# Lecanyu/SparsifyPoseGraph

Measured on AMD Instinct MI355X. Metric: nodes_marginalized_per_s, higher is better.
Workload: dtype f64

## Files before the change

sparsifyposegraph_amd/csrc/spg_graph_impl.h:

```cpp
#pragma once
#include <algorithm>
#include <atomic>
#include <chrono>
#include <cmath>
#include <cstdio>
#include <cstdlib>
#include <cstring>
#include <set>
#include <string>
#include <thread>
#if defined(__linux__)
#include <pthread.h>
#include <sched.h>
#endif
#include <unistd.h>
#include <unordered_map>
#include <unordered_set>
#include <vector>
#include "../../include/spg.h"
#include "spg_internal.h"

namespace {
inline int pose_stride(int d) { return d == 3 ? 3 : 7; }
inline int info_len(int d) { return d * (d + 1) / 2; }
// ... 86 lines not shown
    spg_backend be{};
    bool is_hip = false;
    int rank = 0, nranks = 1;
    void *rccl = nullptr;
    int tag_counter = 0;
    int linear_solver = 0;
    double pcg_rel_tol = 0;
    int pcg_max_iter = 0;
    spg_pcg_stats pcg_stats{};
    spg::StreamPort *sim_port = nullptr;
    char err[768] = {0};
};

struct GEdge {
    int64_t off;
    int64_t key;
    int32_t len;
    int32_t vtx[2];
    int16_t nv;
    int8_t kind;
    uint8_t alive;
};

struct RoundBlanket {
    int32_t root;
    int32_t n_remove;
    int32_t vbeg = 0, nv = 0;
    int32_t ebeg = 0, ne = 0;
    int32_t rank = 0;
    int32_t owner = -1;
    spg_blanket_desc desc{};
};

struct BlanketLog { int32_t root_id, round, status, info; double kld, min_gap; };

struct Batch {
    std::vector<RoundBlanket> rb;
    std::vector<int32_t> rb_verts, rb_edges;
    std::vector<spg_blanket_desc> h_blk;
    std::vector<int64_t> h_vpo;
    std::vector<spg_edge_ref> h_er;
    std::vector<int32_t> h_ev;
    std::vector<int64_t> chunk_hdr;
    spg_round_info rinfo{};
    bool round_open = false;
    bool used_mailbox = false;
// ... 22 lines not shown
        if (vdirect_ok) return (id >= 0 && (size_t)id < vdirect.size()) ? vdirect[(size_t)id] : -1;
        auto it = vidx.find(id);
        return it == vidx.end() ? -1 : it->second;
    }
    std::vector<uint8_t> valive;
    std::vector<int64_t> vpose;
    struct AdjEnt { int32_t eid, other; operator int32_t() const { return eid; } };
    struct SVtx {
        int32_t nown;
        int32_t own[4];
        int32_t slot;
    };
    struct alignas(64) VRec {
        InlVec<AdjEnt, 7> adj;
        SVtx s;
        int32_t id, pad_;
        int64_t pose;
        char spare_[24];
        VRec() { s.nown = 0; s.slot = -1; id = 0; pad_ = 0; pose = 0; }
    };
    std::vector<VRec> vr;
    std::vector<InlVec<struct OwnRefT, 3>> vown;
    std::vector<int32_t> cst;
    std::vector<GEdge> edges;
    std::vector<int32_t> everts;
    int n_live_v = 0, n_live_e = 0;
    void *dev = nullptr;
    int64_t cap = 0, used = 0;
    HostMirror host;
    int64_t dev_synced = 0;
    int64_t stale_lo = 0, stale_hi = 0;
    bool active = false;
    spg_options opts{};
    int rank = 0, nranks = 1;
    std::vector<int32_t> pending;
    size_t pend_head = 0;
    std::vector<uint8_t> in_set;
    static constexpr int NB = 8;
    Batch bt[NB];
    Batch *B = &bt[0];
    struct Owner { int32_t batch, off, len; uint32_t gen; };
    using OwnRef = OwnRefT;
    std::vector<Owner> owners;
    std::vector<int32_t> owner_free, transient;
    std::vector<int32_t> Dpool;
    int shard_threshold = -1;
    int round_no = 0, launch_seq = 0;
    bool pipelined = false;
    spg_marg_stats stats{};
    double tr_age = 0, tr_wait = 0, tr_first = 0; long tr_n = 0;
    std::vector<BlanketLog> log;
    std::vector<double> hdr_buf;
    std::thread sub_thread;
    static constexpr uint32_t SUBQ = 8;
    bool sub_active = false;
    struct alignas(64) SubShared {
        alignas(64) std::atomic<uint32_t> tail{0};
        alignas(64) Batch *q[SUBQ] = {nullptr};
        alignas(64) std::atomic<uint32_t> head{0};
        alignas(64) double seconds = 0;
// ... 3 lines not shown
    std::vector<int32_t> live_rank;
    long n_mutations = 0, live_rank_stamp = -1;
    int64_t next_key = 0, key_base = 0;
    static constexpr int64_t kKeyStride = 65536;
    std::vector<int32_t> lpos;
    std::vector<int32_t> vstamp, estamp;
    int32_t stamp = 0;
    std::vector<int32_t> ocnt;
    std::vector<int32_t> lidx;
    std::vector<int32_t> s_newpending, s_B, s_centres, s_Dv, s_tmp, s_work, s_seen, s_hit, s_vix;
    std::vector<double> s_cost;
    std::vector<int> s_first;
    static constexpr int kSOwn = 4, kSMaxV = 16, kSMaxE = 44;
    struct SSlot {
        int32_t pos, root, nv, ne, n_new_max, tag, logi, bell;
        int32_t launched;
        int32_t npend, pend[3];
        int32_t mcell;
        int64_t new_off, out_off;
        int32_t verts[kSMaxV];
        int32_t edges[kSMaxE];
    };
    std::vector<SSlot> sslots;
    std::vector<int32_t> s_free, s_fifo, s_fin, s_woken, s_ready, wl_next, wl_stable, wl_done;
    int64_t unsorted_from = -1;
    bool layout_diverged = false;
    int stream_emulation = -1;
    int stream_disabled = 0;
};

static inline const int32_t *edge_verts(const spg_graph *g, const GEdge &e) {
    return e.nv == 2 ? e.vtx : g->everts.data() + e.vtx[0];
}

inline int set_err(spg_ctx *c, int code, const char *fmt, const char *a = "") {
    if (c) snprintf(c->err, sizeof c->err, fmt, a);
    return code;
}

int sync_host(spg_graph *g);
int sync_device(spg_graph *g);
void canonicalize_edge_order(spg_graph *g);
#pragma GCC visibility push(hidden)
int arena_ensure(spg_graph *g, int64_t need);
int add_edge_idx(spg_graph *g, int kind, int nv, const int32_t *vix, int64_t off, int32_t len, int64_t key = -1);
void quiesce_submission(spg_graph *g);
int stream_marginalize(spg_graph *g, bool *started = nullptr);
#pragma GCC visibility pop

namespace {
inline void next_stamp(spg_graph *g) {
    if (g->vstamp.size() < g->vid.size()) g->vstamp.resize(g->vid.size(), 0);
    if (g->estamp.size() < g->edges.size()) g->estamp.resize(g->edges.size(), 0);
    g->stamp++;
}

inline void mark_stale(spg_graph *g, int64_t lo, int64_t hi) {
    if (g->stale_hi <= g->stale_lo) { g->stale_lo = lo; g->stale_hi = hi; }
    else { g->stale_lo = std::min(g->stale_lo, lo); g->stale_hi = std::max(g->stale_hi, hi); }
}

inline void copy_backend_error(spg_ctx *c) { snprintf(c->err, sizeof c->err, "%s", spg::hip_backend_error(&c->be)); }

enum MailState { MAIL_NOT_YET = 0, MAIL_READY = 1, MAIL_FINAL = 2 };
inline MailState mail_state(double word, double tag) {
    return word == SPG_READY_WORD(tag) ? MAIL_READY : word == SPG_FINAL_WORD(tag) ? MAIL_FINAL : MAIL_NOT_YET;
}

inline bool out_record_well_formed(const double *rec, const spg_blanket_desc &bd, int nv) {
// ... 81 lines not shown
```

sparsifyposegraph_amd/csrc/spg_hip_backend.cpp:

```cpp
#include <hip/hip_runtime.h>
#include <atomic>
#include <chrono>
#include <cstdio>
#include <cstdlib>
#include <cstring>
#include <vector>
#include <algorithm>
#include "../../include/spg.h"
#include "spg_blanket_layout.hpp"
#include "spg_hip_buffers.hpp"
#include "spg_internal.h"
#include "spg_round_plan.hpp"

namespace spg {

#define HIPCHK(x) do { hipError_t e_ = (x); if (e_ != hipSuccess) { snprintf(err, (size_t)512, "%s:%d %s -> %s", __FILE__, __LINE__, #x, hipGetErrorString(e_)); return SPG_EHIP; } } while (0)

namespace {

bool env_is(const char *name, char c) { const char *e = getenv(name); return e && e[0] == c; }

struct HipBackend {
    int device = 0;
    char err[512] = {0};
// ... 5 lines not shown
        PinnedBuf stage;
        bool busy = false;
        RoundPlan plan;
        hipEvent_t done = nullptr, wait_ev = nullptr;
        DevBuf bar;
        std::vector<const volatile double *> finals;
        double final_word = 0;
        DevBuf pkt;
        bool stream_dirty = false;
        std::vector<Timed> pending;
        std::vector<std::pair<hipEvent_t, hipEvent_t>> pool;
        double prof_ms = 0, prof_bytes = 0;
        long long prof_launches = 0, prof_blankets = 0;
    };
    static constexpr int NSLOT = 8;
    Slot slots[NSLOT];
    struct Worker {
        hipStream_t stream = nullptr;
        DevBuf qmem;
        DevBuf ticket;
        WorkQ *q() const { return (WorkQ *)qmem.p; }
        hipEvent_t ev_a = nullptr, ev_b = nullptr;
        bool running = false, disabled = false;
        int D = 0, alg = 0;
        unsigned long long tail = 0;
        double bytes = 0;
        long long blankets = 0;
        int bells = 1, lazy = 0;
        int wgs = 256;
        std::chrono::steady_clock::time_point last_push;
    } worker;
    int batches_in_call = 0;
    DevBuf st_pkt;
    PinnedBuf st_mail;
    int worker_cooldown = 0;
    double prof_big_ms = 0, prof_big_flops = 0;
    long long prof_big_count = 0;
    int prof_big_nmax = 0;
    double prof_worker_ms = 0, prof_worker_bytes = 0;
    long long prof_worker_runs = 0, prof_worker_blankets = 0;
    int lds_limit = 160 * 1024;
    bool large_bar = false;
    std::atomic<int> n_launches{0};
    const bool force_one_wave = env_is("SPG_ONE_WAVE", '1');
    const bool worker_env = !env_is("SPG_WORKER", '0');
    const bool worker_stamp = env_is("SPG_WORKER_STAMP", '1');
// ... 92 lines not shown
        t.bytes = B.bytes; t.blankets = nblocks;
    }
    const hipEvent_t stop = timed ? t.b : S.done;
    if (int rc = hip_blanket_launch(B.variant, S.stream, timed ? t.a : nullptr, stop, ka, nblocks, B.lds, err, sizeof err)) {
        if (timed) S.pool.push_back({t.a, t.b});
        return rc;
    }
    if (timed) S.pending.push_back(t);
    S.wait_ev = stop;
    n_launches++;
    S.stream_dirty = true;
    return 0;
}

inline void bar_fence() {
    std::atomic_thread_fence(std::memory_order_release);
#if defined(__x86_64__)
    __builtin_ia32_sfence();
#endif
}

int HipBackend::worker_start(int D, int alg) {
    Worker &W = worker;
    if (W.running && W.D == D && W.alg == alg) {
        if (std::chrono::duration<double>(std::chrono::steady_clock::now() - W.last_push).count() < 1.0) return 0;
    }
    if (W.running) if (int rc = worker_stop()) return rc;
    if (!W.stream) {
        HIPCHK(hipStreamCreateWithFlags(&W.stream, hipStreamNonBlocking));
        HIPCHK(hipEventCreate(&W.ev_a));
        HIPCHK(hipEventCreate(&W.ev_b));
        if (W.qmem.alloc_fine(sizeof(WorkQ)) != hipSuccess) { (void)hipGetLastError(); W.disabled = true; return 1; }
        HIPCHK(W.ticket.alloc(64));
        const char *e = getenv("SPG_WORKER_WGS");
        if (e && atoi(e) > 0) W.wgs = atoi(e);
        if ((e = getenv("SPG_WORKER_BELLS")) && atoi(e) >= 1 && atoi(e) <= kBells) W.bells = atoi(e);
        if ((e = getenv("SPG_WORKER_LAZY")) && atoi(e) >= 0) W.lazy = atoi(e);
    }
    WorkQ *q = W.q();
    for (int c = 0; c < W.bells; c++) q->tail[c * kBellStride] = 0;
    q->stop = 0;
    bar_fence();
    W.tail = 0; W.bytes = 0; W.blankets = 0;
    HIPCHK(hipMemsetAsync(W.ticket.p, 0, 64, W.stream));
    Layout L = make_layout(D, 128, kWorkerMaxN / D, 1, alg, SPG_TOPO_TREE, 0);
    const size_t lds = (size_t)(L.small_doubles + L.mat_doubles) * 8;
    const long long idle_ticks = 10LL * 100000000LL;
    if (int rc = hip_worker_launch(D, W.wgs, lds, W.stream, W.ev_a, W.ev_b, q, (unsigned long long *)W.ticket.p, idle_ticks, W.bells, W.lazy, err, sizeof err)) return rc;
    W.running = true; W.D = D; W.alg = alg;
    W.last_push = std::chrono::steady_clock::now();
    n_launches++;
    return 0;
}

int HipBackend::worker_stop() {
    Worker &W = worker;
    if (!W.running) return 0;
    W.q()->stop = 1;
    bar_fence();
    HIPCHK(hipStreamSynchronize(W.stream));
    W.running = false;
    if (profiling) {
        float ms = 0;
        if (hipEventElapsedTime(&ms, W.ev_a, W.ev_b) == hipSuccess) {
            prof_worker_ms += ms; prof_worker_bytes += W.bytes; prof_worker_runs++; prof_worker_blankets += W.blankets;
        }
    }
    return 0;
}

int HipBackend::push_to_worker(Slot &S, const spg_round_desc *rd, void *arena) {
    const spg_options &o = *rd->opts;
    const int D = o.pose_dim;
    const size_t n_push = (size_t)rd->count;
    bool fine = true;
    if (int rc = ensure_fine(S.pkt, n_push * (size_t)kPktWords * 8, (size_t)512 * kPktWords * 8, &fine)) return rc;
    if (!fine) worker.disabled = true;
    if (int rc = ensure_pinned(S.mail, (size_t)rd->mail_len * 8, true)) return rc;
    if (worker.disabled) return 1;
    if (int wrc = worker_start(D, SPG_ALG_NFR)) return wrc;
    Worker &W = worker;
    WorkQ *q = W.q();
    unsigned long long *pbase = (unsigned long long *)S.pkt.p;
    const double *hmail = (const double *)S.mail.h;
// ... 200 lines not shown
        double secs = 0, flops = 0;
        const int info_bits = (rd->opts->flags & SPG_FLAG_GLC_KLD) ? SPG_INFO_GLC_KLD_SKIPPED : 0;
        if (int brc = hip_big_glc_dense((void *)S.stream, g.in, m, k, Nm, bd.new_off, orec, bd.n_new_max, rd->tag, info_bits, &secs, &flops, err, sizeof err)) return brc;
        prof_big_ms += 1e3 * secs; prof_big_flops += flops; prof_big_count++;
        prof_big_nmax = std::max(prof_big_nmax, D * (k + m));
        S.wait_ev = nullptr;
        S.stream_dirty = true;
    }
    return 0;
}

int HipBackend::run_round(void *arena, const spg_round_desc *rd) {
    if (rd->count <= 0) return 0;
    Slot &S = slots[rd->slot & (NSLOT - 1)];
    const spg_options &o = *rd->opts;
    if (o.pose_dim != 3 && o.pose_dim != 6) return SPG_EINVAL;
    if (int rc = make_current()) return rc;
    if (S.busy) if (int rc = wait_slot(S)) return rc;
    drain_profile(S);
    S.busy = true;
    PlanConfig cfg;
    cfg.lds_limit = lds_limit; cfg.force_one_wave = force_one_wave; cfg.large_bar = large_bar;
    cfg.worker_enabled = worker_env && !worker.disabled; cfg.force_big = force_big; cfg.profiling = profiling;
    const WorkerState ws{++batches_in_call, worker_cooldown, worker.running};
    plan_worker(rd, cfg, ws, S.plan);
    worker_cooldown = S.plan.cooldown;
    if (S.plan.to_worker) {
        const int rc = push_to_worker(S, rd, arena);
        if (rc <= 0) return rc;
    }
    if (int rc = worker_stop()) return rc;
    if (int rc = plan_launch(rd, cfg, S.plan, err, sizeof err)) return rc;
    Staged sd{};
    if (int rc = stage_descriptors(S, rd, sd)) return rc;
    double *mail_dev = nullptr;
    if (rd->mail_len > 0) {
        if (int rc = ensure_pinned(S.mail, (size_t)rd->mail_len * 8, true)) return rc;
        mail_dev = (double *)S.mail.d;
    }
    KArgs ka;
    ka.arena = (double *)arena;
    ka.blk = (const spg_blanket_desc *)(sd.base + sd.o_blk);
    ka.vpo = (const int64_t *)(sd.base + sd.o_vpo);
    ka.er = (const spg_edge_ref *)(sd.base + sd.o_er);
    ka.ev = (const int32_t *)(sd.base + sd.o_ev);
    ka.list = nullptr;
    ka.mail = mail_dev;
// ... 176 lines not shown
    if (wrc) return wrc;
    if (hb->worker.disabled) return 1;
    hb->batches_in_call += 3;
    out->pkt = (unsigned long long *)hb->st_pkt.p;
    out->q = hb->worker.q();
    out->tail = hb->worker.tail;
    out->bells = hb->worker.bells;
    out->h_mail = (const double *)hb->st_mail.h;
    out->d_mail = (unsigned long long)(uintptr_t)hb->st_mail.d;
    out->mail_stride = mail_stride;
    out->slots = slots;
    return 0;
}

void hip_stream_close(spg_backend *b, const StreamPort *port, double alg_bytes, long long blankets) {
    HipBackend *hb = (HipBackend *)b->user;
    if (!hb || !port) return;
    hb->worker.tail = port->tail;
    hb->worker.bytes += alg_bytes;
    hb->worker.blankets += blankets;
    hb->worker.last_push = std::chrono::steady_clock::now();
}

}
```

sparsifyposegraph_amd/csrc/spg_host_rounds.cpp:

```cpp
#include "spg_graph_impl.h"

static void closed_neighbourhood(spg_graph *g, int32_t v, std::vector<int32_t> &out) {
    next_stamp(g);
    out.clear();
    out.push_back(v);
    g->vstamp[v] = g->stamp;
    for (int32_t eid : g->vr[v].adj) {
        const GEdge &e = g->edges[eid];
        for (int i = 0; i < e.nv; i++) {
            int32_t u = edge_verts(g, e)[i];
            if (g->vstamp[u] != g->stamp) { g->vstamp[u] = g->stamp; out.push_back(u); }
        }
    }
}

static void extended_blanket(spg_graph *g, int32_t root, std::vector<int32_t> &verts, std::vector<int32_t> &picked) {
    auto byid = [g](int32_t a, int32_t b) { return g->vid[a] < g->vid[b]; };
    std::set<int32_t, decltype(byid)> ret(byid), pk(byid);
    std::vector<int32_t> tmp;
    closed_neighbourhood(g, root, tmp);
    ret.insert(tmp.begin(), tmp.end());
    pk.insert(root);
    for (auto it = ret.begin(); it != ret.end(); ++it) {
        int32_t v = *it;
// ... 182 lines not shown
                    }
                }
            }
            if (Dv.size() > DCAP) { stop = true; continue; }
            {
                int32_t off = (int32_t)g->Dpool.size();
                g->Dpool.insert(g->Dpool.end(), Dv.begin(), Dv.end());
                g->transient.push_back(reg(-1, off, (int32_t)Dv.size()));
            }
            static const int pat_inflight = [] { const char *e = getenv("SPG_PATIENCE"); return e ? atoi(e) : 16; }();
            size_t patience = inflight ? pat_inflight + bt.rb.size() / 16 : 48 + bt.rb.size() / 8;
            if (++consec > patience || n_deferred > 256 + 2 * bt.rb.size()) stop = true;
            PT(3);
        }
    }
    {
        size_t nd = newpending.size();
        size_t nh = pos - nd;
        for (size_t i = 0; i < nd; i++) g->pending[nh + i] = newpending[i];
        g->pend_head = nh;
    }
}

extern "C" int spg_graph_marginalize_begin(spg_graph *g, const int32_t *which, int n, const spg_options *opts, int rank, int nranks) {
    if (!g || !opts || (n > 0 && !which) || nranks < 1 || rank < 0 || rank >= nranks) return SPG_EINVAL;
    if (g->active) return set_err(g->ctx, SPG_ESTATE, "marginalize already in progress");
    if (opts->pose_dim != g->d) return set_err(g->ctx, SPG_EINVAL, "pose_dim mismatch");
    g->opts = *opts;
    g->rank = rank; g->nranks = nranks;
    g->pending.clear();
    g->pend_head = 0;
    g->in_set.assign(g->vid.size(), 0);
    g->lpos.assign(g->vid.size(), -1);
    for (int i = 0; i < n; i++) {
        const int32_t vi = g->index_of(which[i]);
        if (vi < 0 || !g->valive[vi])
            return set_err(g->ctx, SPG_EINVAL, "vertex needs to exist in order to be marginalized");
        if (g->in_set[vi]) continue;
        g->in_set[vi] = 1;
        g->lpos[vi] = (int32_t)g->pending.size();
        g->pending.push_back(vi);
    }
    g->key_base = g->next_key;
    g->next_key = g->key_base + ((int64_t)g->pending.size() + 1) * spg_graph::kKeyStride;
    if (g->cap < g->used * 5 / 2 + (1 << 16)) if (int rc = arena_ensure(g, g->used * 3 + (1 << 20))) return rc;
    if (int rc = sync_device(g)) return rc;
    g->active = true;
    for (int i = 0; i < spg_graph::NB; i++) { g->bt[i].round_open = false; g->bt[i].slot = i; }
    g->B = &g->bt[0];
    g->round_no = 0;
    g->launch_seq = 0;
    g->pipelined = false;
    g->stats = spg_marg_stats{};
    g->log.clear();
    return 0;
}

extern "C" int spg_graph_set_shard_threshold(spg_graph *g, int min_blankets) {
    if (!g) return SPG_EINVAL;
    g->shard_threshold = min_blankets < 0 ? -1 : min_blankets;
    return 0;
}

static bool shard_pays(const spg_graph *g, const Batch &bt) {
    const int B = (int)bt.rb.size(), nr = g->nranks;
    if (nr <= 1 || B == 0) return false;
    if (g->shard_threshold >= 0) return B >= g->shard_threshold;
    const int d = g->d;
    double t_sum = 0, t_max = 0, bytes = 0;
    for (const RoundBlanket &r : bt.rb) {
        const double n = (double)d * (r.nv - r.n_remove), nm = (double)d * r.n_remove;
        const double tb = 45e-6 * std::pow(std::max(1.0, n / 24.0), 2.5);
        const double lds = 8.0 * (3 * n * n + nm * nm + nm * n) + 4096.0;
        const double per_cu = lds > 160.0 * 1024 ? 1.0 : std::min(6.0, std::floor(160.0 * 1024 / lds));
        t_sum += tb / (256.0 * per_cu);
        t_max = std::max(t_max, tb);
        int32_t nn, nvv; int64_t nl;
        new_edge_budget(g->opts, d, r.nv - r.n_remove, nn, nvv, nl);
// ... 344 lines not shown
            return set_err(g->ctx, SPG_EHIP, "%s", msg);
        }
        const int64_t key0 = g->key_base + (int64_t)g->lpos[r.root] * spg_graph::kKeyStride;
        for_each_new_edge(rec, n_new, bd.n_new_max, [&](int e, int kind, int64_t rel, int32_t len, int nv, const double *lv) {
            vix.resize(nv);
            for (int i = 0; i < nv; i++) vix[i] = rverts[(int)lv[i]];
            add_edge_idx(g, kind, nv, vix.data(), bd.new_off + rel, len, key0 + e);
            g->stats.n_new_edges++;
        });
        PT(10);
    }
    bt.round_open = false;
    release_batch_owners(g, bt);
    g->stats.n_rounds = g->round_no;
    g->stats.host_seconds += now_s() - t1;
    g->stats.commit_seconds += now_s() - t1;
    return 0;
}

extern "C" int spg_graph_marginalize_end(spg_graph *g, spg_marg_stats *stats) {
    if (!g || !g->active) return SPG_ESTATE;
    submission_stop(g);
    g->active = false;
    for (int i = 0; i < spg_graph::NB; i++) (void)harvest_kld(g, g->bt[i]);
    for (int i = 0; i < spg_graph::NB; i++) { g->bt[i].round_open = false; release_batch_owners(g, g->bt[i]); g->bt[i].rb.clear(); }
    for (int32_t oid : g->transient) owner_release(g, oid);
    g->transient.clear();
    g->B = &g->bt[0];
    if (g->ctx->is_hip) (void)spg::hip_backend_end_of_call(&g->ctx->be);
    if (g->tr_n && getenv("SPG_TRACE"))
        fprintf(stderr, "spg trace: %ld batches; per batch: launch call -> commit start %.1f us, wait for the ready words %.1f us (launch call -> first blanket ready %.1f us)\n",
                g->tr_n, 1e6 * g->tr_age / g->tr_n, 1e6 * g->tr_wait / g->tr_n, 1e6 * g->tr_first / g->tr_n);
    g->tr_n = 0; g->tr_age = g->tr_wait = g->tr_first = 0;
    if (g->ctx->is_hip) g->stats.n_launches = spg::hip_backend_launches(&g->ctx->be);
#ifdef SPG_SCHED_PROF
    if (getenv("SPG_SCHED_PROF")) {
        const char *nm[12] = {"neighbourhood", "owner scan", "select:reg", "defer", "-", "select:sort", "select:edges", "commit:log", "commit:rm edges", "commit:rm verts", "commit:add", "prepare"};
        for (int i = 0; i < 12; i++) { fprintf(stderr, "sched %-14s %10llu calls %8.3f Mcycles\n", nm[i], prof_n[i], prof_t[i] * 1e-6); prof_t[i] = prof_n[i] = 0; }
    }
#endif
    if (stats) *stats = g->stats;
    return g->stats.n_bad_status ? SPG_EBLANKET : 0;
}

static Batch *oldest_open_batch(spg_graph *g) {
    Batch *o = nullptr;
// ... 7 lines not shown
    for (size_t i = from; i < to; i++) {
        RoundBlanket r = a.rb[i];
        int32_t vb = (int32_t)b.rb_verts.size(), eb = (int32_t)b.rb_edges.size();
        b.rb_verts.insert(b.rb_verts.end(), a.rb_verts.begin() + r.vbeg, a.rb_verts.begin() + r.vbeg + r.nv);
        b.rb_edges.insert(b.rb_edges.end(), a.rb_edges.begin() + r.ebeg, a.rb_edges.begin() + r.ebeg + r.ne);
        r.vbeg = vb; r.ebeg = eb;
        if (r.owner >= 0) { g->owners[r.owner].batch = bidx; g->owners[r.owner].off = vb; }
        b.rb.push_back(r);
    }
}

extern "C" int spg_graph_marginalize(spg_graph *g, const int32_t *which, int n, const spg_options *opts, spg_marg_stats *stats) {
    return spg_graph_marginalize_ranks(g, which, n, opts, 0, 1, nullptr, nullptr, stats);
}

extern "C" int spg_graph_marginalize_ranks(spg_graph *g, const int32_t *which, int n, const spg_options *opts, int rank, int nranks,
                                           spg_exchange_fn exchange, void *exchange_user, spg_marg_stats *stats) {
    if (!g) return SPG_EINVAL;
    const bool builtin = nranks > 1 && !exchange;
    if (builtin && (!g->ctx->rccl || g->ctx->nranks != nranks || g->ctx->rank != rank))
        return set_err(g->ctx, SPG_EINVAL, "spg_graph_marginalize_ranks: no exchange callback and the context has no matching RCCL communicator (spg_ctx_create_ranks)");
    int launches0 = (g && g->ctx->is_hip) ? spg::hip_backend_launches(&g->ctx->be) : 0;
    const double t_call = now_s();
    int rc = spg_graph_marginalize_begin(g, which, n, opts, rank, nranks);
    if (rc) return rc;
    const double t_begun = now_s();
    const char *env = getenv("SPG_NO_PIPELINE");
    g->pipelined = g->ctx->be.synchronize_slot && g->ctx->be.mailbox_slot && !(env && env[0] == '1');
    int stream_rc = 1;
    if (nranks == 1 && !exchange) stream_rc = stream_marginalize(g);
    else if (nranks > 1) {
        bool independent = g->layout_diverged;
        if (!independent && g->shard_threshold < 0) {
            const std::vector<int32_t> saved = g->pending;
            g->B = &g->bt[0];
            schedule_round(g);
            independent = !g->bt[0].rb.empty() && !shard_pays(g, g->bt[0]);
            release_batch_owners(g, g->bt[0]);
            g->bt[0].rb.clear(); g->bt[0].rb_verts.clear(); g->bt[0].rb_edges.clear();
            for (int32_t oid : g->transient) owner_release(g, oid);
            g->transient.clear();
            g->pending = saved;
            g->pend_head = 0;
        }
        if (independent) {
            const int rank0 = g->rank, nranks0 = g->nranks;
            g->rank = 0; g->nranks = 1;
            bool started = false;
            stream_rc = stream_marginalize(g, &started);
            if (started || g->layout_diverged) g->layout_diverged = true;
            else { g->rank = rank0; g->nranks = nranks0; }
        }
    }
    if (stream_rc <= 0) {
        const double t_streamed = now_s();
        int rc2 = spg_graph_marginalize_end(g, stats);
        if (getenv("SPG_TRACE")) fprintf(stderr, "spg trace: marginalize: begin %.3f ms, stream %.3f ms, end %.3f ms\n", 1e3 * (t_begun - t_call), 1e3 * (t_streamed - t_begun), 1e3 * (now_s() - t_streamed));
        if (stats && g->ctx->is_hip) stats->n_launches -= launches0;
        return stream_rc < 0 ? stream_rc : rc2;
    }
    auto do_exchange = [&](Batch &b) -> int {
        if (!b.rinfo.exchange) return 0;
        double tx = now_s();
        int erc = g->ctx->be.synchronize(g->ctx->be.user);
        if (erc) return erc;
        erc = builtin ? spg_allgather_region(g->ctx, g->dev, b.rinfo.region_off, b.rinfo.chunk_len)
                      : exchange(exchange_user, g->dev, b.rinfo.region_off, b.rinfo.chunk_len, g->nranks, g->rank);
        g->stats.n_exchanged++;
        g->stats.exchanged_bytes += 8.0 * (double)b.rinfo.chunk_len * g->nranks;
        g->stats.exchange_seconds += now_s() - tx;
        return erc;
    };
    if (!g->pipelined) {
        for (;;) {
            rc = spg_graph_round_prepare(g, nullptr);
            if (rc <= 0) break;
// ... 88 lines not shown
```

sparsifyposegraph_amd/csrc/spg_host_stream.cpp:

```cpp
#include "spg_graph_impl.h"

#if defined(__x86_64__)
#include <x86intrin.h>
static inline uint64_t ticks_now() { return __rdtsc(); }
#else
static inline uint64_t ticks_now() { return (uint64_t)(now_s() * 1e9); }
#endif

namespace {
enum : uint8_t { SV_WAITING = 0, SV_STABLE = 1, SV_INFLIGHT = 2, SV_DONE = 3 };
constexpr int kStreamSlots = 2048;
constexpr int kStreamMailStride = 8;

__attribute__((always_inline)) inline void unregister_blanket(spg_graph *g, const int32_t s) {
    const spg_graph::SSlot &sl = g->sslots[s];
    spg_graph::VRec *const vr = g->vr.data();
    for (int i = 0; i < sl.nv; i++) {
        spg_graph::SVtx &sx = vr[sl.verts[i]].s;
        for (int j = 0; j < sx.nown; j++) if (sx.own[j] == s) { sx.own[j] = sx.own[--sx.nown]; break; }
    }
}

struct Streamer {
    spg_graph *g;
    const bool emulate;
    const int D, ps, rec;
    const int32_t P;
    int32_t cursor = 0;
    int32_t prefetched_to = 0;
    int32_t n_done = 0, n_inflight = 0, pending_bell = 0, bell_no = 0;
    bool fallback = false;
    int32_t cap_wait = -1;
    uint64_t t_idle = 0;

    Streamer(spg_graph *g_, bool emu) : g(g_), emulate(emu), D(g_->d), ps(g_->ps), rec(g_->rec), P((int32_t)g_->pending.size()), arena_dev(g_->dev) {}

    struct SvView { spg_graph::VRec *vr; spg_graph::SVtx &operator[](int32_t i) const { return vr[i].s; } };

    long n_exam = 0, n_park[8] = {0};
    const bool prof = [] { const char *e = getenv("SPG_STREAM_PROF"); return e && e[0] == '1'; }();
    uint64_t pt[8] = {0}, pn[8] = {0}, pt_last = 0;
    inline void P0() { if (prof) pt_last = ticks_now(); }
    inline void P1(int i) { if (prof) { const uint64_t n = ticks_now(); pt[i] += n - pt_last; pn[i]++; pt_last = n; } }
    void park(std::vector<int32_t> &heads, int32_t on, int32_t p) { g->wl_next[p] = heads[on]; heads[on] = p; }
    void wake(std::vector<int32_t> &heads, int32_t on) {
        for (int32_t p = heads[on]; p >= 0;) { const int32_t nx = g->wl_next[p]; g->s_woken.push_back(p); p = nx; }
        heads[on] = -1;
    }

    static inline int find(const int32_t *X, const int nX, const int32_t y) { for (int i = 0; i < nX; i++) if (X[i] == y) return i; return -1; }
    static inline void adj_remove(InlVec<spg_graph::AdjEnt, 7> &av, const int32_t eid) {
        for (size_t j = 0; j < av.size(); j++) if (av[j].eid == eid) { av[j] = av.back(); av.pop_back(); break; }
    }
    inline void set_pend(spg_graph::SSlot &sl, const int32_t *X, const int nX) {
        const int32_t *const cst = g->cst.data();
        sl.npend = 0;
        for (int i = 1; i < nX; i++) if (cst[X[i]] >= 0) { if (sl.npend == 3) { sl.npend = -1; break; } sl.pend[sl.npend++] = X[i]; }
    }
    __attribute__((always_inline)) inline void register_blanket(const int32_t s, const int32_t p, const int32_t *X, const int nX) {
        const SvView sv{g->vr.data()};
        spg_graph::SSlot &sl = g->sslots[s];
        sl.pos = p; sl.root = X[0]; sl.nv = nX;
        memcpy(sl.verts, X, sizeof(int32_t) * (size_t)nX);
        set_pend(sl, X, nX);
        for (int i = 0; i < nX; i++) { spg_graph::SVtx &sx = sv[X[i]]; sx.own[sx.nown++] = s; }
    }

    void reserve(const int32_t p, const int32_t *X, const int nX) {
// ... 324 lines not shown
            uint32_t q = poll_seq;
            for (int n = 0; q != launch_seq && n < 12; q++) {
                if (cell_slot[q & mask] < 0) continue;
                __builtin_prefetch((const void *)(port.h_mail + (size_t)(q & mask) * (size_t)port.mail_stride));
                n++;
            }
        }
    }

    struct Helper {
        static constexpr uint32_t RQ = 4096;
        alignas(64) std::atomic<uint32_t> launches{0};
        alignas(64) std::atomic<uint32_t> r_tail{0};
        alignas(64) std::atomic<int> stop{0};
        alignas(64) uint32_t r_head = 0;
        std::vector<double> rq;
        std::vector<uint32_t> cell_tag;
        char pad_[64];
    } hp;
    bool helper = false;
    std::thread helper_thread;
    std::vector<const double *> ready_rec;

    void helper_main() {
        const uint32_t mask = (uint32_t)(port.slots - 1);
        std::vector<uint8_t> pend((size_t)port.slots, 0);
        uint32_t head = 0, seen = 0, r_tail = 0;
        unsigned n = 0;
        while (!hp.stop.load(std::memory_order_acquire)) {
            const uint32_t lp = hp.launches.load(std::memory_order_acquire);
            while (seen != lp) { pend[seen & mask] = 1; seen++; }
            while (head != seen && !pend[head & mask]) head++;
            const int giveup = (++n & 15) ? 10 : 1 << 20;
            bool got = false;
            scan_mailbox(head, seen, giveup,
                         [&](uint32_t cell, double &tagd) -> int32_t {
                             if (!pend[cell]) return -1;
                             tagd = (double)hp.cell_tag[cell];
                             return (int32_t)cell;
                         },
                         [&](uint32_t q, int32_t cell, bool final) {
                             double *e = hp.rq.data() + (size_t)(r_tail & (Helper::RQ - 1)) * 8;
                             memcpy(e, port.h_mail + (size_t)cell * (size_t)port.mail_stride, 64);
                             e[5] = (double)(2.0 * (double)q + (final ? 1.0 : 0.0));
                             r_tail++;
                             pend[cell] = 0;
                             got = true;
                         });
            if (got) hp.r_tail.store(r_tail, std::memory_order_release);
        }
    }
    void take_helper_results() {
        const uint32_t rt = hp.r_tail.load(std::memory_order_acquire);
        const uint32_t mask = (uint32_t)(port.slots - 1);
        ready_rec.clear();
        while (hp.r_head != rt) {
            const double *e = hp.rq.data() + (size_t)(hp.r_head & (Helper::RQ - 1)) * 8;
            __builtin_prefetch(e + 8); __builtin_prefetch(e + 16);
            const uint32_t q = (uint32_t)((uint64_t)e[5] >> 1);
            const int32_t s = cell_slot[q & mask];
            g->s_ready.push_back(s);
            ready_rec.push_back(e);
            cell_slot[q & mask] = -2;
            __builtin_prefetch(&g->sslots[s]); __builtin_prefetch((const char *)&g->sslots[s] + 64); __builtin_prefetch((const char *)&g->sslots[s] + 128);
            hp.r_head++;
        }
    }
    bool helper_start() {
#if defined(__linux__)
        static const bool pin = [] { const char *e = getenv("SPG_PIN_THREADS"); return !(e && e[0] == '0'); }();
        if (!pin || sched_getaffinity(0, sizeof old_mask, &old_mask) != 0) return false;
        const int cpu = sched_getcpu();
        int cand = -1;
        for (int d = 1; cpu >= 0 && d < 8 && cand < 0; d++) {
            const int c = (cpu & ~7) | ((cpu + d) & 7);
            if (c < CPU_SETSIZE && CPU_ISSET(c, &old_mask)) cand = c;
        }
        if (cand < 0) return false;
        cpu_set_t one; CPU_ZERO(&one); CPU_SET(cpu, &one);
        if (sched_setaffinity(0, sizeof one, &one) != 0) return false;
        repin = true;
        hp.rq.resize((size_t)Helper::RQ * 8);
        hp.cell_tag.assign((size_t)port.slots, 0);
        helper = true;
        helper_thread = std::thread([this] { helper_main(); });
        CPU_ZERO(&one); CPU_SET(cand, &one);
        (void)pthread_setaffinity_np(helper_thread.native_handle(), sizeof one, &one);
        return true;
#else
        return false;
#endif
    }
    void helper_stop() {
        if (!helper) return;
        hp.stop.store(1, std::memory_order_release);
        helper_thread.join();
        helper = false;
#if defined(__linux__)
        if (repin) (void)sched_setaffinity(0, sizeof old_mask, &old_mask);
#endif
    }
#if defined(__linux__)
    cpu_set_t old_mask;
    bool repin = false;
#endif

    size_t fifo_head = 0;
    uint64_t rng;
// ... 152 lines not shown
        const double s_begin = now_s();
        last_progress = t_begin;
        for (;;) {
            if (int r = take_results()) return r;
            const bool got = !ready.empty();
            if (got && idle_since) { t_idle += ticks_now() - idle_since; idle_since = 0; }
            commit_ready();
            examine_woken();
            late_results();
            advance_cursor(got);
            ring();
            if (n_done == P) break;
            if (fallback && n_inflight == 0) break;
            if (got || cursor < P) { last_progress = ticks_now(); continue; }
            if (int r = idle_check()) { if (r < 0) return r; break; }
        }
        if (int r = drain()) return r;
        account(t_begin, s_begin);
        return 0;
    }
};
}

int stream_marginalize(spg_graph *g, bool *started) {
    const spg_options &o = g->opts;
    if (started) *started = false;
    static const bool env_off = [] { const char *e = getenv("SPG_STREAM"); return e && e[0] == '0'; }();
    spg::StreamPort *const sim = g->ctx->is_hip ? nullptr : g->ctx->sim_port;
    const bool emulate = !g->ctx->is_hip && !sim;
    if (env_off || g->stream_disabled) return 1;
    if (emulate && g->stream_emulation < 0) return 1;
    if (g->nranks != 1 || o.algorithm != SPG_ALG_NFR || o.topology != SPG_TOPO_TREE || o.lin_point != SPG_LIN_GLOBAL || o.flags != 0) return 1;
    const int32_t P = (int32_t)g->pending.size();
    if (P < (emulate ? 1 : 64)) return 1;
    Streamer S(g, emulate);
    if (sim) {
        if (sim->slots < kStreamSlots || sim->mail_stride < kStreamMailStride) return 1;
        S.port = *sim;
    } else if (!emulate) {
        int prc = spg::hip_stream_open(&g->ctx->be, g->d, kStreamSlots, kStreamMailStride, &S.port);
        if (prc < 0) { copy_backend_error(g->ctx); return prc; }
        if (prc > 0) return 1;
    }
    const size_t V = g->vid.size();
    if (g->cst.size() < V) g->cst.resize(V, -1);
    for (int32_t p = 0; p < P; p++) { g->cst[g->pending[p]] = (p << 2) | SV_WAITING; g->vr[g->pending[p]].s.nown = 0; }
    g->wl_next.assign((size_t)P, -1); g->wl_stable.assign((size_t)P, -1); g->wl_done.assign((size_t)P, -1);
    if (g->sslots.size() < (size_t)kStreamSlots) g->sslots.resize(kStreamSlots);
    g->s_free.clear();
    for (int s = kStreamSlots - 1; s >= 0; s--) g->s_free.push_back(s);
    g->s_fifo.clear(); g->s_fin.clear(); g->s_woken.clear(); g->s_ready.clear();
    next_stamp(g);
    if (g->lidx.size() < V) g->lidx.resize(V, -1);
    if ((int64_t)g->host.size() < g->cap) g->host.resize((size_t)g->cap);
    S.rng = 0x9E3779B97F4A7C15ULL ^ ((uint64_t)(g->stream_emulation > 0 ? g->stream_emulation : 1) * 0xD1B54A32D192ED03ULL);
    const int64_t used0 = g->used;
    if (started) *started = true;
    if (g->unsorted_from < 0) g->unsorted_from = (int64_t)g->edges.size();
    if (!emulate) S.cell_slot.assign((size_t)S.port.slots, -1);
    static const int want_helper = [] { const char *e = getenv("SPG_STREAM_THREADS"); return e ? atoi(e) : 0; }();
    if (!emulate && (want_helper == 2 || (want_helper == 0 && !sim)) && P >= 4096) (void)S.helper_start();
    const double t_setup = now_s();
    const int rc = S.run();
    S.helper_stop();
    const double t_ran = now_s();
    if (sim) sim->tail = S.port.tail;
    else if (!emulate) spg::hip_stream_close(&g->ctx->be, &S.port, S.alg_bytes, (long long)S.n_done);
    if (g->used > used0) {
        g->dev_synced = g->used;
        if (!emulate && !sim) mark_stale(g, used0, g->used);
        else {
            if (int r = g->ctx->be.download(g->ctx->be.user, g->host.data() + used0, (char *)g->dev + used0 * 8, g->used - used0)) return r;
        }
    }
    g->stats.n_rounds = S.bell_no;
    g->round_no = S.bell_no;
    size_t left = 0;
    for (int32_t p = 0; p < P; p++) {
        const int32_t v = g->pending[p];
        spg_graph::SVtx &sq = g->vr[v].s;
        const int vst = g->cst[v] & 3;
        if (vst == SV_STABLE) unregister_blanket(g, sq.slot);
        const bool done = vst == SV_DONE;
        g->cst[v] = -1; sq.nown = 0;
        if (!done) g->pending[left++] = v;
    }
    g->pending.resize(left);
    g->pend_head = 0;
    if (getenv("SPG_TRACE")) {
        fprintf(stderr, "spg trace: streaming driver: run %.3f ms, tear-down %.3f ms\n", 1e3 * (t_ran - t_setup), 1e3 * (now_s() - t_ran));
        fprintf(stderr, "spg trace: streaming driver: %d list entries, %d committed in %d doorbells, %zu left to the batch driver (examined up to entry %d)\n",
                P, S.n_done, S.bell_no, left, S.cursor);
        fprintf(stderr, "spg trace: streaming driver: %ld examinations; parked on: earlier neighbour %ld, own blanket %ld, two shared vertices %ld, waiting member of a touching blanket %ld, waiting 2-hop neighbour %ld\n",
                S.n_exam, S.n_park[0], S.n_park[1], S.n_park[2], S.n_park[3], S.n_park[4]);
    }
    if (rc) return rc;
    return left ? 1 : 0;
}

extern "C" int spg_debug_set_stream_port(spg_ctx *c, void *port) {
    if (!c || c->is_hip) return SPG_EINVAL;
    c->sim_port = (spg::StreamPort *)port;
    return 0;
}

extern "C" int spg_graph_set_stream_emulation(spg_graph *g, int seed) {
    if (!g) return SPG_EINVAL;
    g->stream_disabled = seed <= -2;
    g->stream_emulation = seed < 0 ? -1 : seed;
    return 0;
}
```

sparsifyposegraph_amd/csrc/spg_internal.h:

```cpp
#pragma once
#include <cstddef>
#include <cstdint>
#include "../../include/spg.h"

namespace spg {

int hip_backend_create(int device, spg_backend *out, char *errbuf, size_t errlen);
void hip_backend_destroy(spg_backend *b);
void *hip_backend_stream(spg_backend *b);
const char *hip_backend_error(spg_backend *b);
int hip_backend_launches(spg_backend *b);
int hip_backend_device(spg_backend *b);
void hip_backend_profile(spg_backend *b, int enable);
void hip_backend_profile_read(spg_backend *b, double *ms, double *bytes, long long *launches, long long *blankets);
void hip_backend_profile_read_worker(spg_backend *b, double *ms, double *bytes, long long *runs, long long *blankets);
void hip_backend_profile_read_big(spg_backend *b, double *ms, double *flops, long long *count, int *nmax);
int hip_backend_end_of_call(spg_backend *b);

constexpr int kQCap = 16384;
constexpr int kPktHdr = 13;
constexpr int kPktWords = 192;
constexpr int kPktStride = 64;
constexpr int kWorkerMaxN = 36;
constexpr int kBells = 16, kBellStride = 512;
struct WorkQ {
    unsigned long long stop;
    unsigned long long pad[7];
    unsigned long long tail[kBells * kBellStride];
    unsigned long long item[kQCap];
};

struct StreamPort {
    unsigned long long *pkt = nullptr;
    WorkQ *q = nullptr;
    unsigned long long tail = 0;
    int bells = 1;
    const double *h_mail = nullptr;
    unsigned long long d_mail = 0;
    int mail_stride = 0, slots = 0;
};
int hip_stream_open(spg_backend *b, int D, int slots, int mail_stride, StreamPort *out);
void hip_stream_close(spg_backend *b, const StreamPort *port, double alg_bytes, long long blankets);

struct BlanketVariant;
struct KArgs;
#pragma GCC visibility push(hidden)
int hip_blanket_launch(const BlanketVariant &v, void *stream, void *ev_start, void *ev_stop, const KArgs &ka, int nblocks, size_t lds_bytes,
                       char *err, size_t errlen);
int hip_worker_launch(int D, int grid, size_t lds_bytes, void *stream, void *ev_start, void *ev_stop, WorkQ *q, unsigned long long *ticket,
                      long long idle_ticks, int bells, int lazy, char *err, size_t errlen);
int hip_local_point_launch(int D, void *stream, int count, const double *arena, double *lpose, const spg_blanket_desc *blk, const int64_t *vpo,
                           const spg_edge_ref *er, const int32_t *ev, const int32_t *list, const int64_t *lp_off, int32_t *flag, char *err, size_t errlen);
#pragma GCC visibility pop

struct DenseGraphIn {
    int D = 0, nv = 0, ne = 0;
    const int32_t *pos = nullptr;
    const int64_t *vpo = nullptr;
    const int32_t *rowptr = nullptr;
    const int32_t *inc = nullptr;
    const spg_edge_ref *er = nullptr;
    const int32_t *ev = nullptr;
    int64_t n_ev = 0;
    const void *dev_arena = nullptr;
};
// ... 36 lines not shown
    double *ws;
    int64_t ws_stride;
    double *mail;
    int64_t mail_base;
    int topology, lin_point, tag;
    int lds_doubles;
    int eig_jacobi;
    int ip_untiled;
    double chord_ratio;
};
constexpr int kIpMaxVars = 8400;
int nfr_ip_pattern_size(int topology, double chord_ratio, int k);
int64_t nfr_ip_workspace(int D, int k, int m, int E, int closed, int64_t *hot);
int hip_nfr_ip_launch(void *stream, int D, IpArgs a, int count, int n_closed, int64_t hot_max);

int rccl_get_unique_id(void *id_out, char *err, size_t errlen);
int rccl_comm_create(int device, int rank, int nranks, const void *unique_id, void **handle, char *err, size_t errlen);
int rccl_allgather_f64(void *handle, void *arena, int64_t region_off, int64_t chunk_len, void *stream, char *err, size_t errlen);
void rccl_comm_destroy(void *handle);

}

extern "C" int spg_debug_set_stream_port(spg_ctx *ctx, void *stream_port);
extern "C" int spg_debug_la(int op, int M, int N, int K, int flags, int mode, double *A, int ra, int lda, double *B, int rb, int ldb, double *C, int rc, int ldc, int *ok);
extern "C" int spg_debug_bsr_bench(spg_graph *g, int32_t fixed_id, int reps, double *out);
```

Before: 3.105 million.

## Skip per-call batch bookkeeping on streaming path and overlap worker stop

When the streaming marginalizer will take the call, begin now marks pending vertices directly in the stream state array, and the in_set/lpos arrays are built only if work is left over for the batched fallback. The streaming setup starts the helper thread before opening the HIP stream, keeps the three worklists in one reused buffer cleared with memset, and avoids resetting nown for every vertex. After a fully completed run it signals the device worker to stop asynchronously instead of waiting for a later stop. These changes target per-call host setup and teardown costs. In exchange they add lazy-state flags and cleanup paths that must keep cst and nown consistent on failures.

```diff
diff --git a/sparsifyposegraph_amd/csrc/spg_graph_impl.h b/sparsifyposegraph_amd/csrc/spg_graph_impl.h
--- a/sparsifyposegraph_amd/csrc/spg_graph_impl.h
+++ b/sparsifyposegraph_amd/csrc/spg_graph_impl.h
@@ -132,6 +132,8 @@
     uint8_t alive;
 };
 
+enum : uint8_t { SV_WAITING = 0, SV_STABLE = 1, SV_INFLIGHT = 2, SV_DONE = 3 };
+
 struct RoundBlanket {
     int32_t root;
     int32_t n_remove;
@@ -200,6 +202,7 @@
     std::vector<VRec> vr;
     std::vector<InlVec<struct OwnRefT, 3>> vown;
     std::vector<int32_t> cst;
+    bool cst_listed = false;
     std::vector<GEdge> edges;
     std::vector<int32_t> everts;
     int n_live_v = 0, n_live_e = 0;
@@ -214,6 +217,7 @@
     std::vector<int32_t> pending;
     size_t pend_head = 0;
     std::vector<uint8_t> in_set;
+    bool batch_state = false;
     static constexpr int NB = 8;
     Batch bt[NB];
     Batch *B = &bt[0];
@@ -263,7 +267,9 @@
         int32_t edges[kSMaxE];
     };
     std::vector<SSlot> sslots;
-    std::vector<int32_t> s_free, s_fifo, s_fin, s_woken, s_ready, wl_next, wl_stable, wl_done;
+    std::vector<int32_t> s_free, s_fifo, s_fin, s_woken, s_ready;
+    std::vector<int32_t> wl_store;
+    int32_t *wl_next = nullptr, *wl_stable = nullptr, *wl_done = nullptr;
     int64_t unsorted_from = -1;
     bool layout_diverged = false;
     int stream_emulation = -1;
@@ -286,6 +292,8 @@
 int arena_ensure(spg_graph *g, int64_t need);
 int add_edge_idx(spg_graph *g, int kind, int nv, const int32_t *vix, int64_t off, int32_t len, int64_t key = -1);
 void quiesce_submission(spg_graph *g);
+void build_batch_state(spg_graph *g);
+bool stream_takes_call(const spg_graph *g, int32_t P);
 int stream_marginalize(spg_graph *g, bool *started = nullptr);
 #pragma GCC visibility pop
 
diff --git a/sparsifyposegraph_amd/csrc/spg_hip_backend.cpp b/sparsifyposegraph_amd/csrc/spg_hip_backend.cpp
--- a/sparsifyposegraph_amd/csrc/spg_hip_backend.cpp
+++ b/sparsifyposegraph_amd/csrc/spg_hip_backend.cpp
@@ -51,6 +51,7 @@
         WorkQ *q() const { return (WorkQ *)qmem.p; }
         hipEvent_t ev_a = nullptr, ev_b = nullptr;
         bool running = false, disabled = false;
+        bool stopping = false;
         int D = 0, alg = 0;
         unsigned long long tail = 0;
         double bytes = 0;
@@ -189,7 +190,7 @@
 
 int HipBackend::worker_start(int D, int alg) {
     Worker &W = worker;
-    if (W.running && W.D == D && W.alg == alg) {
+    if (W.running && !W.stopping && W.D == D && W.alg == alg) {
         if (std::chrono::duration<double>(std::chrono::steady_clock::now() - W.last_push).count() < 1.0) return 0;
     }
     if (W.running) if (int rc = worker_stop()) return rc;
@@ -214,7 +215,7 @@
     const size_t lds = (size_t)(L.small_doubles + L.mat_doubles) * 8;
     const long long idle_ticks = 10LL * 100000000LL;
     if (int rc = hip_worker_launch(D, W.wgs, lds, W.stream, W.ev_a, W.ev_b, q, (unsigned long long *)W.ticket.p, idle_ticks, W.bells, W.lazy, err, sizeof err)) return rc;
-    W.running = true; W.D = D; W.alg = alg;
+    W.running = true; W.stopping = false; W.D = D; W.alg = alg;
     W.last_push = std::chrono::steady_clock::now();
     n_launches++;
     return 0;
@@ -223,10 +224,12 @@
 int HipBackend::worker_stop() {
     Worker &W = worker;
     if (!W.running) return 0;
-    W.q()->stop = 1;
-    bar_fence();
+    if (!W.stopping) {
+        W.q()->stop = 1;
+        bar_fence();
+    }
     HIPCHK(hipStreamSynchronize(W.stream));
-    W.running = false;
+    W.running = false; W.stopping = false;
     if (profiling) {
         float ms = 0;
         if (hipEventElapsedTime(&ms, W.ev_a, W.ev_b) == hipSuccess) {
@@ -473,7 +476,7 @@
     PlanConfig cfg;
     cfg.lds_limit = lds_limit; cfg.force_one_wave = force_one_wave; cfg.large_bar = large_bar;
     cfg.worker_enabled = worker_env && !worker.disabled; cfg.force_big = force_big; cfg.profiling = profiling;
-    const WorkerState ws{++batches_in_call, worker_cooldown, worker.running};
+    const WorkerState ws{++batches_in_call, worker_cooldown, worker.running && !worker.stopping};
     plan_worker(rd, cfg, ws, S.plan);
     worker_cooldown = S.plan.cooldown;
     if (S.plan.to_worker) {
@@ -696,4 +699,12 @@
     hb->worker.last_push = std::chrono::steady_clock::now();
 }
 
-}
+void hip_stream_stop(spg_backend *b) {
+    HipBackend *hb = (HipBackend *)b->user;
+    if (!hb || !hb->worker.running || hb->worker.stopping) return;
+    hb->worker.q()->stop = 1;
+    bar_fence();
+    hb->worker.stopping = true;
+}
+
+}
diff --git a/sparsifyposegraph_amd/csrc/spg_host_rounds.cpp b/sparsifyposegraph_amd/csrc/spg_host_rounds.cpp
--- a/sparsifyposegraph_amd/csrc/spg_host_rounds.cpp
+++ b/sparsifyposegraph_amd/csrc/spg_host_rounds.cpp
@@ -228,7 +228,16 @@
     }
 }
 
-extern "C" int spg_graph_marginalize_begin(spg_graph *g, const int32_t *which, int n, const spg_options *opts, int rank, int nranks) {
+void build_batch_state(spg_graph *g) {
+    if (g->batch_state) return;
+    g->in_set.assign(g->vid.size(), 0);
+    g->lpos.assign(g->vid.size(), -1);
+    const int32_t P = (int32_t)g->pending.size();
+    for (int32_t p = 0; p < P; p++) { g->in_set[g->pending[p]] = 1; g->lpos[g->pending[p]] = p; }
+    g->batch_state = true;
+}
+
+static int marginalize_begin(spg_graph *g, const int32_t *which, int n, const spg_options *opts, int rank, int nranks, bool may_stream) {
     if (!g || !opts || (n > 0 && !which) || nranks < 1 || rank < 0 || rank >= nranks) return SPG_EINVAL;
     if (g->active) return set_err(g->ctx, SPG_ESTATE, "marginalize already in progress");
     if (opts->pose_dim != g->d) return set_err(g->ctx, SPG_EINVAL, "pose_dim mismatch");
@@ -236,21 +245,42 @@
     g->rank = rank; g->nranks = nranks;
     g->pending.clear();
     g->pend_head = 0;
-    g->in_set.assign(g->vid.size(), 0);
-    g->lpos.assign(g->vid.size(), -1);
+    const bool lazy = may_stream && stream_takes_call(g, n);
+    g->batch_state = false;
+    g->cst_listed = false;
+    if (lazy) {
+        if (g->cst.size() < g->vid.size()) g->cst.resize(g->vid.size(), -1);
+    } else {
+        g->in_set.assign(g->vid.size(), 0);
+        g->lpos.assign(g->vid.size(), -1);
+        g->batch_state = true;
+    }
+    auto fail = [&](int rc) {
+        if (lazy) for (int32_t v : g->pending) g->cst[v] = -1;
+        g->pending.clear();
+        return rc;
+    };
+    int32_t *const cst = g->cst.data();
     for (int i = 0; i < n; i++) {
         const int32_t vi = g->index_of(which[i]);
         if (vi < 0 || !g->valive[vi])
-            return set_err(g->ctx, SPG_EINVAL, "vertex needs to exist in order to be marginalized");
-        if (g->in_set[vi]) continue;
-        g->in_set[vi] = 1;
-        g->lpos[vi] = (int32_t)g->pending.size();
+            return fail(set_err(g->ctx, SPG_EINVAL, "vertex needs to exist in order to be marginalized"));
+        const int32_t p = (int32_t)g->pending.size();
+        if (lazy) {
+            if (cst[vi] >= 0) continue;
+            cst[vi] = (p << 2) | SV_WAITING;
+        } else {
+            if (g->in_set[vi]) continue;
+            g->in_set[vi] = 1;
+            g->lpos[vi] = p;
+        }
         g->pending.push_back(vi);
     }
     g->key_base = g->next_key;
     g->next_key = g->key_base + ((int64_t)g->pending.size() + 1) * spg_graph::kKeyStride;
-    if (g->cap < g->used * 5 / 2 + (1 << 16)) if (int rc = arena_ensure(g, g->used * 3 + (1 << 20))) return rc;
-    if (int rc = sync_device(g)) return rc;
+    if (g->cap < g->used * 5 / 2 + (1 << 16)) if (int rc = arena_ensure(g, g->used * 3 + (1 << 20))) return fail(rc);
+    if (int rc = sync_device(g)) return fail(rc);
+    g->cst_listed = lazy;
     g->active = true;
     for (int i = 0; i < spg_graph::NB; i++) { g->bt[i].round_open = false; g->bt[i].slot = i; }
     g->B = &g->bt[0];
@@ -260,6 +290,10 @@
     g->stats = spg_marg_stats{};
     g->log.clear();
     return 0;
+}
+
+extern "C" int spg_graph_marginalize_begin(spg_graph *g, const int32_t *which, int n, const spg_options *opts, int rank, int nranks) {
+    return marginalize_begin(g, which, n, opts, rank, nranks, false);
 }
 
 extern "C" int spg_graph_set_shard_threshold(spg_graph *g, int min_blankets) {
@@ -650,6 +684,10 @@
     if (!g || !g->active) return SPG_ESTATE;
     submission_stop(g);
     g->active = false;
+    if (g->cst_listed) {
+        for (size_t p = g->pend_head; p < g->pending.size(); p++) g->cst[g->pending[p]] = -1;
+        g->cst_listed = false;
+    }
     for (int i = 0; i < spg_graph::NB; i++) (void)harvest_kld(g, g->bt[i]);
     for (int i = 0; i < spg_graph::NB; i++) { g->bt[i].round_open = false; release_batch_owners(g, g->bt[i]); g->bt[i].rb.clear(); }
     for (int32_t oid : g->transient) owner_release(g, oid);
@@ -703,7 +741,7 @@
         return set_err(g->ctx, SPG_EINVAL, "spg_graph_marginalize_ranks: no exchange callback and the context has no matching RCCL communicator (spg_ctx_create_ranks)");
     int launches0 = (g && g->ctx->is_hip) ? spg::hip_backend_launches(&g->ctx->be) : 0;
     const double t_call = now_s();
-    int rc = spg_graph_marginalize_begin(g, which, n, opts, rank, nranks);
+    int rc = marginalize_begin(g, which, n, opts, rank, nranks, nranks == 1 && !exchange);
     if (rc) return rc;
     const double t_begun = now_s();
     const char *env = getenv("SPG_NO_PIPELINE");
@@ -733,6 +771,7 @@
             else { g->rank = rank0; g->nranks = nranks0; }
         }
     }
+    if (stream_rc > 0) build_batch_state(g);
     if (stream_rc <= 0) {
         const double t_streamed = now_s();
         int rc2 = spg_graph_marginalize_end(g, stats);
diff --git a/sparsifyposegraph_amd/csrc/spg_host_stream.cpp b/sparsifyposegraph_amd/csrc/spg_host_stream.cpp
--- a/sparsifyposegraph_amd/csrc/spg_host_stream.cpp
+++ b/sparsifyposegraph_amd/csrc/spg_host_stream.cpp
@@ -8,7 +8,6 @@
 #endif
 
 namespace {
-enum : uint8_t { SV_WAITING = 0, SV_STABLE = 1, SV_INFLIGHT = 2, SV_DONE = 3 };
 constexpr int kStreamSlots = 2048;
 constexpr int kStreamMailStride = 8;
 
@@ -42,8 +41,8 @@
     uint64_t pt[8] = {0}, pn[8] = {0}, pt_last = 0;
     inline void P0() { if (prof) pt_last = ticks_now(); }
     inline void P1(int i) { if (prof) { const uint64_t n = ticks_now(); pt[i] += n - pt_last; pn[i]++; pt_last = n; } }
-    void park(std::vector<int32_t> &heads, int32_t on, int32_t p) { g->wl_next[p] = heads[on]; heads[on] = p; }
-    void wake(std::vector<int32_t> &heads, int32_t on) {
+    void park(int32_t *heads, int32_t on, int32_t p) { g->wl_next[p] = heads[on]; heads[on] = p; }
+    void wake(int32_t *heads, int32_t on) {
         for (int32_t p = heads[on]; p >= 0;) { const int32_t nx = g->wl_next[p]; g->s_woken.push_back(p); p = nx; }
         heads[on] = -1;
     }
@@ -414,9 +413,9 @@
     std::thread helper_thread;
     std::vector<const double *> ready_rec;
 
-    void helper_main() {
-        const uint32_t mask = (uint32_t)(port.slots - 1);
-        std::vector<uint8_t> pend((size_t)port.slots, 0);
+    void helper_main(const int slots) {
+        const uint32_t mask = (uint32_t)(slots - 1);
+        std::vector<uint8_t> pend((size_t)slots, 0);
         uint32_t head = 0, seen = 0, r_tail = 0;
         unsigned n = 0;
         while (!hp.stop.load(std::memory_order_acquire)) {
@@ -425,7 +424,7 @@
             while (head != seen && !pend[head & mask]) head++;
             const int giveup = (++n & 15) ? 10 : 1 << 20;
             bool got = false;
-            scan_mailbox(head, seen, giveup,
+            if (head != seen) scan_mailbox(head, seen, giveup,
                          [&](uint32_t cell, double &tagd) -> int32_t {
                              if (!pend[cell]) return -1;
                              tagd = (double)hp.cell_tag[cell];
@@ -458,7 +457,7 @@
             hp.r_head++;
         }
     }
-    bool helper_start() {
+    bool helper_start(const int slots) {
 #if defined(__linux__)
         static const bool pin = [] { const char *e = getenv("SPG_PIN_THREADS"); return !(e && e[0] == '0'); }();
         if (!pin || sched_getaffinity(0, sizeof old_mask, &old_mask) != 0) return false;
@@ -473,9 +472,9 @@
         if (sched_setaffinity(0, sizeof one, &one) != 0) return false;
         repin = true;
         hp.rq.resize((size_t)Helper::RQ * 8);
-        hp.cell_tag.assign((size_t)port.slots, 0);
+        hp.cell_tag.assign((size_t)slots, 0);
         helper = true;
-        helper_thread = std::thread([this] { helper_main(); });
+        helper_thread = std::thread([this, slots] { helper_main(slots); });
         CPU_ZERO(&one); CPU_SET(cand, &one);
         (void)pthread_setaffinity_np(helper_thread.native_handle(), sizeof one, &one);
         return true;
@@ -674,30 +673,36 @@
 };
 }
 
-int stream_marginalize(spg_graph *g, bool *started) {
+bool stream_takes_call(const spg_graph *g, const int32_t P) {
     const spg_options &o = g->opts;
-    if (started) *started = false;
     static const bool env_off = [] { const char *e = getenv("SPG_STREAM"); return e && e[0] == '0'; }();
+    const bool emulate = !g->ctx->is_hip && !g->ctx->sim_port;
+    if (env_off || g->stream_disabled) return false;
+    if (emulate && g->stream_emulation < 0) return false;
+    if (g->nranks != 1 || o.algorithm != SPG_ALG_NFR || o.topology != SPG_TOPO_TREE || o.lin_point != SPG_LIN_GLOBAL || o.flags != 0) return false;
+    return P >= (emulate ? 1 : 64);
+}
+
+static int stream_run(spg_graph *g, bool *started) {
+    const int32_t P = (int32_t)g->pending.size();
     spg::StreamPort *const sim = g->ctx->is_hip ? nullptr : g->ctx->sim_port;
     const bool emulate = !g->ctx->is_hip && !sim;
-    if (env_off || g->stream_disabled) return 1;
-    if (emulate && g->stream_emulation < 0) return 1;
-    if (g->nranks != 1 || o.algorithm != SPG_ALG_NFR || o.topology != SPG_TOPO_TREE || o.lin_point != SPG_LIN_GLOBAL || o.flags != 0) return 1;
-    const int32_t P = (int32_t)g->pending.size();
-    if (P < (emulate ? 1 : 64)) return 1;
     Streamer S(g, emulate);
+    int slots = kStreamSlots;
     if (sim) {
         if (sim->slots < kStreamSlots || sim->mail_stride < kStreamMailStride) return 1;
         S.port = *sim;
-    } else if (!emulate) {
-        int prc = spg::hip_stream_open(&g->ctx->be, g->d, kStreamSlots, kStreamMailStride, &S.port);
-        if (prc < 0) { copy_backend_error(g->ctx); return prc; }
-        if (prc > 0) return 1;
+        slots = sim->slots;
     }
     const size_t V = g->vid.size();
-    if (g->cst.size() < V) g->cst.resize(V, -1);
-    for (int32_t p = 0; p < P; p++) { g->cst[g->pending[p]] = (p << 2) | SV_WAITING; g->vr[g->pending[p]].s.nown = 0; }
-    g->wl_next.assign((size_t)P, -1); g->wl_stable.assign((size_t)P, -1); g->wl_done.assign((size_t)P, -1);
+    if (!g->cst_listed) {
+        if (g->cst.size() < V) g->cst.resize(V, -1);
+        for (int32_t p = 0; p < P; p++) g->cst[g->pending[p]] = (p << 2) | SV_WAITING;
+        g->cst_listed = true;
+    }
+    if (g->wl_store.size() < 3 * (size_t)P) g->wl_store.resize(3 * (size_t)P);
+    memset(g->wl_store.data(), 0xff, 3 * (size_t)P * sizeof(int32_t));
+    g->wl_next = g->wl_store.data(); g->wl_stable = g->wl_next + P; g->wl_done = g->wl_stable + P;
     if (g->sslots.size() < (size_t)kStreamSlots) g->sslots.resize(kStreamSlots);
     g->s_free.clear();
     for (int s = kStreamSlots - 1; s >= 0; s--) g->s_free.push_back(s);
@@ -706,14 +711,23 @@
     if (g->lidx.size() < V) g->lidx.resize(V, -1);
     if ((int64_t)g->host.size() < g->cap) g->host.resize((size_t)g->cap);
     S.rng = 0x9E3779B97F4A7C15ULL ^ ((uint64_t)(g->stream_emulation > 0 ? g->stream_emulation : 1) * 0xD1B54A32D192ED03ULL);
+    if (!emulate) S.cell_slot.assign((size_t)slots, -1);
+    static const int want_helper = [] { const char *e = getenv("SPG_STREAM_THREADS"); return e ? atoi(e) : 0; }();
+    if (!emulate && (want_helper == 2 || (want_helper == 0 && !sim)) && P >= 4096) (void)S.helper_start(slots);
+    if (!emulate && !sim) {
+        const int prc = spg::hip_stream_open(&g->ctx->be, g->d, kStreamSlots, kStreamMailStride, &S.port);
+        if (prc) {
+            S.helper_stop();
+            if (prc < 0) copy_backend_error(g->ctx);
+            return prc < 0 ? prc : 1;
+        }
+    }
     const int64_t used0 = g->used;
     if (started) *started = true;
     if (g->unsorted_from < 0) g->unsorted_from = (int64_t)g->edges.size();
-    if (!emulate) S.cell_slot.assign((size_t)S.port.slots, -1);
-    static const int want_helper = [] { const char *e = getenv("SPG_STREAM_THREADS"); return e ? atoi(e) : 0; }();
-    if (!emulate && (want_helper == 2 || (want_helper == 0 && !sim)) && P >= 4096) (void)S.helper_start();
     const double t_setup = now_s();
-    const int rc = S.run();
+    int rc = S.run();
+    if (!emulate && !sim && rc == 0 && S.n_done == P) spg::hip_stream_stop(&g->ctx->be);
     S.helper_stop();
     const double t_ran = now_s();
     if (sim) sim->tail = S.port.tail;
@@ -722,21 +736,24 @@
         g->dev_synced = g->used;
         if (!emulate && !sim) mark_stale(g, used0, g->used);
         else {
-            if (int r = g->ctx->be.download(g->ctx->be.user, g->host.data() + used0, (char *)g->dev + used0 * 8, g->used - used0)) return r;
+            const int r = g->ctx->be.download(g->ctx->be.user, g->host.data() + used0, (char *)g->dev + used0 * 8, g->used - used0);
+            if (r && !rc) rc = r;
         }
     }
     g->stats.n_rounds = S.bell_no;
     g->round_no = S.bell_no;
+    if (S.n_done < P) build_batch_state(g);
+    int32_t *const cst = g->cst.data();
     size_t left = 0;
     for (int32_t p = 0; p < P; p++) {
         const int32_t v = g->pending[p];
-        spg_graph::SVtx &sq = g->vr[v].s;
-        const int vst = g->cst[v] & 3;
-        if (vst == SV_STABLE) unregister_blanket(g, sq.slot);
-        const bool done = vst == SV_DONE;
-        g->cst[v] = -1; sq.nown = 0;
-        if (!done) g->pending[left++] = v;
-    }
+        const int vst = cst[v] & 3;
+        if (vst == SV_STABLE) unregister_blanket(g, g->vr[v].s.slot);
+        cst[v] = -1;
+        if (vst != SV_DONE) g->pending[left++] = v;
+    }
+    g->cst_listed = false;
+    if (rc < 0) for (size_t v = 0; v < V; v++) g->vr[v].s.nown = 0;
     g->pending.resize(left);
     g->pend_head = 0;
     if (getenv("SPG_TRACE")) {
@@ -750,6 +767,27 @@
     return left ? 1 : 0;
 }
 
+int stream_marginalize(spg_graph *g, bool *started) {
+    if (started) *started = false;
+    const int rc = stream_takes_call(g, (int32_t)g->pending.size()) ? stream_run(g, started) : 1;
+    if (g->cst_listed) {
+        for (int32_t v : g->pending) g->cst[v] = -1;
+        g->cst_listed = false;
+    }
+    return rc;
+}
+
+extern "C" int spg_debug_stream_state_clean(spg_graph *g) {
+    if (!g) return SPG_EINVAL;
+    if (g->active) return SPG_ESTATE;
+    if (g->cst_listed) return 0;
+    for (size_t v = 0; v < g->vr.size(); v++) {
+        if (g->vr[v].s.nown != 0) return 0;
+        if (v < g->cst.size() && g->cst[v] != -1) return 0;
+    }
+    return 1;
+}
+
 extern "C" int spg_debug_set_stream_port(spg_ctx *c, void *port) {
     if (!c || c->is_hip) return SPG_EINVAL;
     c->sim_port = (spg::StreamPort *)port;
diff --git a/sparsifyposegraph_amd/csrc/spg_internal.h b/sparsifyposegraph_amd/csrc/spg_internal.h
--- a/sparsifyposegraph_amd/csrc/spg_internal.h
+++ b/sparsifyposegraph_amd/csrc/spg_internal.h
@@ -41,6 +41,7 @@
 };
 int hip_stream_open(spg_backend *b, int D, int slots, int mail_stride, StreamPort *out);
 void hip_stream_close(spg_backend *b, const StreamPort *port, double alg_bytes, long long blankets);
+void hip_stream_stop(spg_backend *b);
 
 struct BlanketVariant;
 struct KArgs;
@@ -123,5 +124,6 @@
 }
 
 extern "C" int spg_debug_set_stream_port(spg_ctx *ctx, void *stream_port);
+extern "C" int spg_debug_stream_state_clean(spg_graph *g);
 extern "C" int spg_debug_la(int op, int M, int N, int K, int flags, int mode, double *A, int ra, int lda, double *B, int rb, int ldb, double *C, int rc, int ldc, int *ok);
 extern "C" int spg_debug_bsr_bench(spg_graph *g, int32_t fixed_id, int reps, double *out);
```

New measurement: 3.010 million. -3.1%, worse.
